# infancy/ky

Measured on AMD Instinct MI355X. Metric: Msamples/s (paths*spp), higher is better.
Workload: dtype f32

## Files before the change

ky_amd/csrc/ky_device.hpp:

```cpp
#pragma once
#ifndef __HIPCC_RTC__
#include <hip/hip_runtime.h>
#include <stdint.h>
#endif

#include "ky_scene.hpp"

#define KY_DEV __device__ __forceinline__

#if defined(KY_PROFILE_LANES) || defined(KY_PROFILE_CLOCKS) || defined(KY_MARKS)
#include "ky_measure.hpp"
#else
#define KY_PROBE(k) do { } while (0)
#define KY_CLK(k) do { } while (0)
#endif

namespace kyd {

KY_DEV float rcp(float x) { return __builtin_amdgcn_rcpf(x); }
KY_DEV float rsq(float x) { return __builtin_amdgcn_rsqf(x); }
KY_DEV float fsqrt(float x) { return __builtin_amdgcn_sqrtf(x); }
KY_DEV float sin_rev(float x) { return __builtin_amdgcn_sinf(x); }
KY_DEV float cos_rev(float x) { return __builtin_amdgcn_cosf(x); }
KY_DEV float clamp01f(float x) { return __builtin_amdgcn_fmed3f(x, 0.f, 1.f); }
// ... 838 lines not shown
    const float cos_o = dot(v.normal, wo), cos_i = dot(v.normal, wi);
    abs_cos_i = fabsf(cos_i);
    const bool same = cos_o * cos_i > 0;
    float p = same ? abs_cos_i * K_INV_PI : 0.f;
    scale = same ? K_INV_PI : 0.f;
    const bool phong = B.lobe == LOBE_PHONG;
    col = ld3(phong ? B.m->cs : B.m->c0);
    if (phong) {
        const float cos_alpha = dot(vertex_basis_c(v), wi);
        const float exponent = B.m->exponent;
        const float pe = phong_pow_lobe(cos_alpha, *B.m);
        const float p0 = exponent == 0.f ? 1.f : (exponent > 0.f ? 0.f : K_INF);
        scale = same ? pe * B.m->inv_eta : 0.f;
        p = (cos_alpha > 0.f ? pe : p0) * B.m->phong_pdf_norm;
    }
    const bool nondelta = !bsdf_is_delta(B);
    scale = nondelta ? scale : 0.f;
    pdf = nondelta ? p : 0.f;
}

KY_DEV f3 bsdf_sample_dir_nondelta(const Vertex& v, f3 wo, float u0, float u1, bool* back_dead = nullptr, bool flat_phong = false) {
    const bool phong = v.bsdf.lobe == LOBE_PHONG;
    const float cos_o = dot(v.normal, wo);
    float ang, rad, z = any_f();
    if (phong) {
        z = pow_nonneg(u1, v.bsdf.m->eta);
        rad = fsqrt(1.f - z * z);
        ang = u0;
    } else {
        const float rx = 2.f * u0 - 1, ry = 2.f * u1 - 1;
        const bool xmajor = fabsf(rx) > fabsf(ry);
        rad = xmajor ? rx : ry;
        const float ratio = mul_legacy(xmajor ? ry : rx, rcp(rad));
        ang = xmajor ? 0.125f * ratio : 0.25f - 0.125f * ratio;
    }
    float px = cos_rev(ang) * rad, py = sin_rev(ang) * rad;
    if (!phong) {
        z = __builtin_copysignf(fsqrt(fmaxf(0.f, 1 - px * px - py * py)), cos_o);
    }
    const LobeBasis L = vertex_basis(v);
    f3 wi = L.a * px + L.b * py + L.c * z;
    if (!flat_phong)
    if (phong && cos_o < 0) {
        const float nw = dot(v.normal, wi);
        wi = wi - (2.f * nw) * v.normal;
        if (back_dead) {
            const float cos_alpha = z - 2.f * nw * dot(v.normal, L.c);
            const float pe = phong_pow(cos_alpha, v.bsdf.m->exponent, v.bsdf.m->exp_flags);
            *back_dead = v.bsdf.m->exponent > 0.f && !(cos_alpha > 0.f && pe > 0.f);
        }
    }
    return wi;
}

struct DeltaSample {
    f3 wi;
    float percent;
    float abs_cos;
    bool reflected;
};
KY_DEV DeltaSample bsdf_sample_delta(const Vertex& v, f3 wo, float u0) {
    const DMat& M = *v.bsdf.m;
    const bool glass = v.bsdf.lobe == LOBE_GLASS;
    const float cos_o = dot(v.normal, wo);
    const float eta_t = M.eta, inv_eta = M.inv_eta;
    const bool into = cos_o > 0;
    const float nz = into ? 1.f : -1.f;
    const float ratio = into ? inv_eta : eta_t;
    const float ei = into ? 1.f : eta_t, et = into ? eta_t : 1.f;
    const float cos_theta_i = fminf(fabsf(cos_o), 1.f);
    const float sin_theta_i_sq = fmaxf(0.f, 1 - cos_theta_i * cos_theta_i);
    const float sin_theta_t = ratio * fsqrt(sin_theta_i_sq);
    const bool tir = sin_theta_t >= 1;
    const float cos_theta_t = fsqrt(fmaxf(0.f, 1 - sin_theta_t * sin_theta_t));
    const float r_para = ((et * cos_theta_i) - (ei * cos_theta_t)) * rcp((et * cos_theta_i) + (ei * cos_theta_t));
    const float r_perp = ((ei * cos_theta_i) - (et * cos_theta_t)) * rcp((ei * cos_theta_i) + (et * cos_theta_t));
    const float reflect_percent = (!glass || tir) ? 1.f : (r_para * r_para + r_perp * r_perp) * 0.5f;
    DeltaSample s;
    s.reflected = !glass || u0 < reflect_percent;
    const float k = ratio * cos_theta_i - cos_theta_t;
    const float sw = s.reflected ? -1.f : -ratio, sn = s.reflected ? 2.f * cos_o : k * nz;
    s.wi = wo * sw + v.normal * sn;
    s.percent = s.reflected ? reflect_percent : 1 - reflect_percent;
    s.abs_cos = fabsf(s.reflected ? cos_o : -ratio * cos_o + k * nz);
    return s;
}

KY_DEV BsdfSample bsdf_sample(const Vertex& v, f3 wo, float u0, float u1) {
    BsdfSample s;
    if (bsdf_is_delta(v.bsdf)) {
        const DeltaSample d = bsdf_sample_delta(v, wo, u0);
        s.wi = d.wi;
        s.pdf = d.percent;
        s.f = (ld3(d.reflected ? v.bsdf.m->c0 : v.bsdf.m->c1) * d.percent) * rcp(d.abs_cos);
        s.flags = (d.reflected ? BSDF_REFLECTION : BSDF_TRANSMISSION) | BSDF_SPECULAR;
    } else {
        float abs_cos_i;
        s.wi = bsdf_sample_dir_nondelta(v, wo, u0, u1);
        bsdf_eval_pdf(v, wo, s.wi, s.f, s.pdf, abs_cos_i);
        s.flags = BSDF_REFLECTION | (v.bsdf.lobe == LOBE_PHONG ? BSDF_GLOSSY : BSDF_DIFFUSE);
    }
    return s;
}

struct BsdfContinue {
    f3 wi, weight;
    bool ok, specular;
};
KY_DEV BsdfContinue bsdf_continue(const Vertex& v, f3 wo, float u0, float u1, bool flat_phong = false) {
    BsdfContinue c;
    c.specular = bsdf_is_delta(v.bsdf);
    if (c.specular) {
        const DeltaSample d = bsdf_sample_delta(v, wo, u0);
        c.wi = d.wi;
        c.weight = ld3(d.reflected ? v.bsdf.m->c0 : v.bsdf.m->c1);
        c.ok = ((v.bsdf.m->exp_flags & (d.reflected ? 4 : 8)) != 0) & (d.percent != 0.f);
    } else {
        bool back_dead = false;
        c.wi = bsdf_sample_dir_nondelta(v, wo, u0, u1, &back_dead, flat_phong);
        const float cos_o = dot(v.normal, wo), cos_i = dot(v.normal, c.wi);
        const bool phong = v.bsdf.lobe == LOBE_PHONG;
        const f3 col = ld3(phong ? v.bsdf.m->c1 : v.bsdf.m->c0);
        c.weight = col * (phong ? fabsf(cos_i) : 1.f);
        const bool dead_u1 = phong & !(u1 > 0.f) & (v.bsdf.m->exponent > 0.f);
        c.ok = (cos_o * cos_i > 0) & ((v.bsdf.m->exp_flags & (phong ? 8 : 4)) != 0) & !dead_u1 & !back_dead;
    }
    return c;
}

struct LightSample {
    f3 position, wi, Li;
    float pdf;
    bool lit;
    f3 dir;
    float dist;
};

KY_DEV f3 uniform_sphere_sample(float u0, float u1) {
    const float z = 1 - 2 * u0;
    const float radius = fsqrt(fmaxf(0.f, 1.f - z * z));
    return mk3(radius * cos_rev(u1), radius * sin_rev(u1), z);
}

KY_DEV void shape_sample_position(const DLight& L, float u0, float u1, f3& position, f3& normal, int feat = 0) {
    if ((feat & KY_FEAT_RECT_LIGHTS) || (!(feat & KY_FEAT_SPHERE_LIGHTS) && L.shape_kind == KY_SHAPE_RECTANGLE)) {
        const float4 P = *reinterpret_cast<const float4*>(L.p1), E0 = *reinterpret_cast<const float4*>(L.e0), E1 = *reinterpret_cast<const float4*>(L.e1),
                     N = *reinterpret_cast<const float4*>(L.n);
        position = mk3(P.x, P.y, P.z) + mk3(E0.x, E0.y, E0.z) * u0 + mk3(E1.x, E1.y, E1.z) * u1;
        normal = mk3(N.x, N.y, N.z);
    } else if ((feat & KY_FEAT_SPHERE_LIGHTS) || L.shape_kind == KY_SHAPE_SPHERE) {
        const f3 dir = uniform_sphere_sample(u0, u1);
        position = ld3(L.p1) + L.radius * dir;
        normal = dir;
    } else if (L.shape_kind == KY_SHAPE_TRIANGLE) {
        const float su0 = fsqrt(u0);
        const float bx = 1 - su0, by = u1 * su0;
        position = bx * ld3(L.p1) + by * ld3(L.e0) + (1 - bx - by) * ld3(L.e1);
        normal = ld3(L.n);
    } else {
        const Frame fr = make_frame(ld3(L.n));
        float px, py;
        concentric_disk(u0, u1, px, py);
        position = ld3(L.p1) + L.radius * (fr.s * px + fr.t * py);
        normal = ld3(L.n);
    }
}

KY_DEV void shape_sample_direction(const DLight& L, f3 p, f3 p_normal, float u0, float u1, f3& lposition, f3& lnormal, float& pdf, int feat = 0, bool ipdf = false) {
    const bool sphere = (feat & KY_FEAT_SPHERE_LIGHTS) ? true : ((feat & KY_FEAT_RECT_LIGHTS) == 0 && L.shape_kind == KY_SHAPE_SPHERE);
    const f3 c = ld3(L.p1);
    const float dc2 = length_sq(p - c);
    if (sphere && !(dc2 <= L.radius * L.radius)) {
        const float inv_dist = rsq(dc2);
        const float sin_theta_max = L.radius * inv_dist;
        const float sin_theta_max_sq = sin_theta_max * sin_theta_max;
        const float inv_sin_theta_max = (dc2 * inv_dist) * L.e0[0];
        const float cos_theta_max = fsqrt(fmaxf(0.f, 1 - sin_theta_max_sq));
        float cos_theta = (cos_theta_max - 1) * u0 + 1;
        float sin_theta_sq = 1 - cos_theta * cos_theta;
        if (sin_theta_max_sq < 0.00068523f) {
            sin_theta_sq = sin_theta_max_sq * u0;
            cos_theta = fsqrt(1 - sin_theta_sq);
        }
        const float cos_alpha = sin_theta_sq * inv_sin_theta_max +
                                cos_theta * fsqrt(fmaxf(0.f, 1.f - sin_theta_sq * inv_sin_theta_max * inv_sin_theta_max));
        const float sin_alpha = fsqrt(fmaxf(0.f, 1.f - cos_alpha * cos_alpha));
        const Frame fr = make_frame((c - p) * inv_dist);
        const f3 world_normal = (sin_alpha * cos_rev(u1)) * (-fr.s) + (sin_alpha * sin_rev(u1)) * (-fr.t) + cos_alpha * (-fr.n);
        lposition = c + L.radius * world_normal;
        lnormal = world_normal;
        pdf = ipdf ? 2 * K_PI * (1 - cos_theta_max) : rcp(2 * K_PI * (1 - cos_theta_max));
        return;
    }
    shape_sample_position(L, u0, u1, lposition, lnormal, feat);
    const f3 wv = lposition - p;
    const float d2 = length_sq(wv);
    const f3 wi = wv * rsq(d2);
    const f3 nn = sphere ? p_normal : lnormal;
    if (ipdf) {
        const float r = rsq(d2);
        const float x = (L.area * fabsf(dot(nn, wi))) * (r * r);
        pdf = x > 0.f ? x : K_INF;
        return;
    }
    const float q = L.inv_area * d2 * rcp(fabsf(dot(nn, wi)));
    pdf = __builtin_amdgcn_classf(q, 0x180) ? q : 0.f;
}

KY_DEV float shape_pdf_direction(const DLight& L, const DShapeFull* __restrict__ full, f3 p, f3 p_normal, f3 wi, bool general = true, int feat = 0, bool ipdf = false) {
    const bool sphere = (feat & KY_FEAT_SPHERE_LIGHTS) ? true : ((feat & KY_FEAT_RECT_LIGHTS) == 0 && L.shape_kind == KY_SHAPE_SPHERE);
    const f3 c = ld3(L.p1);
    const float dc2 = length_sq(p - c);
    if (sphere && !(dc2 <= L.radius * L.radius)) {
        const float sin_theta_max_sq = L.radius * L.radius * rcp(dc2);
        const float cos_theta_max = fsqrt(fmaxf(0.f, 1 - sin_theta_max_sq));
        const float x = 2 * K_PI * (1 - cos_theta_max);
        return ipdf ? x : rcp(x);
    }

    const f3 o = offset_ray_origin(p, p_normal, wi);
    float t;
    if (!surf_hit(L.isect, full, o, wi, K_INF, t, general)) return ipdf ? K_INF : 0.f;
    const f3 hp = o + t * wi;
    f3 ln = ld3(L.n);
    if (sphere) ln = normalize(hp - c);
    float pdf = length_sq(p - hp) * rcp(fabsf(dot(ln, wi)) * L.area);
    if (isinf(pdf)) pdf = 0.f;
    return ipdf ? rcp(pdf) : pdf;
}

KY_DEV float env_pdf(float wz) {
    const float z = fminf(fmaxf(wz, -1.f), 1.f);
    const float sin_theta = fsqrt(fmaxf(0.f, 1.f - z * z));
    return sin_theta == 0 ? 0.f : rcp(2 * K_PI * K_PI * sin_theta);
}

KY_DEV LightSample light_sample_Li(const DLight& L, f3 p, f3 p_normal, float u0, float u1, int feat = 0, bool ipdf = false) {
    LightSample s;
    s.lit = true;
    s.dir = any3();
    s.dist = any_f();
    const SceneRef K{nullptr, false, feat};
    if (K.is_area(L.kind)) {
        f3 lposition, lnormal;
        shape_sample_direction(L, p, p_normal, u0, u1, lposition, lnormal, s.pdf, feat, ipdf);
        s.position = lposition;
        const f3 dv = lposition - p;
        const float d2 = length_sq(dv);
        const bool ok = !((ipdf ? __builtin_isinf(s.pdf) : s.pdf == 0) || ((feat & KY_FEAT_RECT_LIGHTS) ? false : d2 == 0));
        const float inv_d = rsq(d2);
        const f3 wi = dv * inv_d;
        s.dir = wi;
        s.dist = d2 * inv_d;
        s.wi = mk3(ok ? wi.x : 0.f, ok ? wi.y : 0.f, ok ? wi.z : 0.f);
        const bool lit = ok & (dot(lnormal, wi) < 0) & !is_black_bits(L.color);
        s.lit = lit;
        s.Li = mk3(lit ? L.color[0] : 0.f, lit ? L.color[1] : 0.f, lit ? L.color[2] : 0.f);
    } else if (K.is_delta(L.kind) && L.kind == KY_LIGHT_POINT) {
        const f3 lp = ld3(L.position);
        const f3 dv = lp - p;
        const float inv_d2 = rcp(length_sq(dv));
        s.position = lp;
        s.wi = dv * fsqrt(inv_d2);
        s.pdf = 1.f;
        s.Li = ld3(L.color) * inv_d2;
    } else if (K.is_delta(L.kind)) {
        s.wi = -ld3(L.direction);
        s.position = p + s.wi * (2 * L.world_radius);
        s.pdf = 1;
        s.Li = ld3(L.color);
    } else {
        s.wi = uniform_sphere_sample(u0, u1);
        s.position = p + s.wi * (2 * L.world_radius);
        s.pdf = env_pdf(s.wi.z);
        s.Li = ld3(L.color);
    }
    return s;
}

KY_DEV float light_pdf_Li(const DLight& L, const DShapeFull* __restrict__ full, f3 p, f3 p_normal, f3 wi, bool general = true, int feat = 0, bool ipdf = false) {
    const SceneRef K{nullptr, false, feat};
    if (K.is_area(L.kind)) return shape_pdf_direction(L, full, p, p_normal, wi, general, feat, ipdf);
    if (K.is_env(L.kind)) return env_pdf(wi.z);
    return 0;
}


KY_DEV f3 surface_emission(const LdsScene& Lds, int surface, f3 normal, f3 wo) {
    const int al = Lds.hit[surface].area_light;
    f3 e = mk3(0, 0, 0);
    if (al >= 0 && dot(normal, wo) > 0) e = mk3(Lds.light_color[al][0], Lds.light_color[al][1], Lds.light_color[al][2]);
    return e;
}

struct RideAlong {
    bool want;
    f3 o, d;
    float t;
    int hs;
};
struct ShadowQueue;
struct SqRay;
KY_DEV void sq_push_bsdf_query(SceneRef S, ShadowQueue& q, bool push, f3 o, f3 d, float tmax, f3 c, unsigned tag);
template <bool MIS, bool PER_LANE = false>
KY_DEV void estimate_by_bsdf(SceneRef S, const LdsScene& Lds, const Vertex& v, f3 wo, int li, float u0, float u1, bool active, f3& acc, f3 w,
                             ShadowQueue* sq = nullptr, f3 beta = f3{0, 0, 0}, float weight = 0.f, unsigned tag = 0, RideAlong* ra = nullptr, const DLight* Lp = nullptr) {
    const DLight& L = light_record<PER_LANE>(S, li, Lp);
    if (PER_LANE) { if (S.is_delta(L.kind)) active = false; } else
    if (S.is_delta(L.kind)) return;
    BsdfSample bs;
    f3 f_cos = any3(), o = any3(), Li = any3();
    bs.wi = any3();
    bs.f = any3();
    bs.pdf = any_f();
    bool live = false, lit = false;
    float t_l = any_f();
    const bool fast = PER_LANE ? ((S.feat & KY_FEAT_CARRIERS) != 0 && (S.feat & (KY_FEAT_SINGLE_AREA | KY_FEAT_SPHERE_LIGHTS)) != 0)
                         : (S.is_area(L.kind) && ((S.feat & KY_FEAT_CARRIERS) || (L.n_carriers >= 0 && S->n_gen == 0)));
    if (fast) {
        const bool act = active && !bsdf_is_delta(v.bsdf);
        if (act) {
            bs.wi = bsdf_sample_dir_nondelta(v, wo, u0, u1, nullptr, S.flat_phong());
            o = offset_ray_origin(v.position, v.normal, bs.wi);
        }
        t_l = K_INF;
        int c = -1;
        bool pending;
        Li = ld3(L.color);
        if (S.feat & KY_FEAT_OWN_CARRIER) {
            const DSurf& R = L.isect;
            float t;
            bool hit;
            if (S.no_par()) {
                const float4 q0 = make_float4(L.aar[0], L.aar[1], L.aar[2], L.aar[3]);
                const float rv = L.aar[4];
                const int ax = L.aar_axis;
                float u_, v_;
                if (ax == 0) {
                    t = (q0.x - o.x) * rcp(bs.wi.x); u_ = (o.y + t * bs.wi.y) - q0.y; v_ = (o.z + t * bs.wi.z) - q0.w;
                    asm volatile("; lamp in an x plane" : "+v"(t), "+v"(u_), "+v"(v_));
                } else if (ax == 1) {
                    t = (q0.x - o.y) * rcp(bs.wi.y); u_ = (o.z + t * bs.wi.z) - q0.y; v_ = (o.x + t * bs.wi.x) - q0.w;
                    asm volatile("; lamp in a y plane" : "+v"(t), "+v"(u_), "+v"(v_));
                } else {
                    t = (q0.x - o.z) * rcp(bs.wi.z); u_ = (o.x + t * bs.wi.x) - q0.y; v_ = (o.y + t * bs.wi.y) - q0.w;
                    asm volatile("; lamp in a z plane" : "+v"(t), "+v"(u_), "+v"(v_));
                }
                hit = (fabsf(u_) <= q0.z) & (fabsf(v_) <= rv) & (t > K_SHAPE_EPS);
            } else {
                hit = par_hit(make_float4(R.f[0], R.f[1], R.f[2], R.f[3]), make_float4(R.f[4], R.f[5], R.f[6], R.f[7]), make_float4(R.f[8], R.f[9], R.f[10], R.f[11]), o, bs.wi, K_INF, t);
            }
            const bool ok = act & hit;
            t_l = ok ? t : t_l;
            c = ok ? L.carrier[0] : c;
            pending = ok && !is_black_bits(L.color);
        } else {
        for (int k = 0; k < L.n_carriers; ++k) {
            float t;
            bool hit;
            if (S.sphere_lights() && k == 0)
                hit = sph_hit(make_float4(L.aar[0], L.aar[1], L.aar[2], L.aar[3]), o, bs.wi, t_l, t, true);
            else
                hit = surf_hit(surf_record<PER_LANE>(S, L.carrier[k]), S->full, o, bs.wi, t_l, t, S.general, S.sphere_lights());
            const bool ok = act & hit;
            t_l = ok ? t : t_l;
            c = ok ? L.carrier[k] : c;
        }
        pending = c >= 0 && !is_black(Li);
        if (pending) {
            const f3 hp = o + t_l * bs.wi;
            pending = dot(hit_normal(Lds.hit[c], hp, bs.wi), bs.wi) < 0;
        }
        }
        if (pending) {
            float abs_cos_i;
            bsdf_eval_pdf(v, wo, bs.wi, bs.f, bs.pdf, abs_cos_i);
            f_cos = bs.f * abs_cos_i;
            live = !(is_black(f_cos) || (MIS ? (bs.pdf <= 0) : (bs.pdf == 0)));
            pending = live;
        }
        if (sq) {
            f3 c = any3();
            if (pending) {
                f3 Lq = (f_cos * Li) * rcp(bs.pdf);
                if (MIS) {
                    float light_pdf;
                    if (L.pdf_from_carrier) {
                        const f3 hp = o + t_l * bs.wi;
                        light_pdf = length_sq(v.position - hp) * rcp(fabsf(dot(ld3(L.n), bs.wi)) * L.area);
                        if (isinf(light_pdf)) light_pdf = 0.f;
                    } else {
                        light_pdf = light_pdf_Li(L, S->full, v.position, v.normal, bs.wi, S.general, S.feat);
                    }
                    Lq = light_pdf > 0 ? (f_cos * Li) * (2.f * rcp(bs.pdf + light_pdf)) : mk3(0, 0, 0);
                }
                c = (Lq * beta) * weight;
                pending = !(c.x == 0.f && c.y == 0.f && c.z == 0.f);
            }
            sq_push_bsdf_query(S, *sq, pending, o, bs.wi, t_l * (1.f - 1e-6f), c, tag);
            return;
        }
        unsigned long long queries = __ballot(pending);
        bool blocked = false;
        if (S.large && S->n_surfaces > 64) {
            KY_PROBE(2);
            if (pending) blocked = trace_any(S, S->occ, o, bs.wi, t_l * (1.f - 1e-6f));
        } else {
            const int lane = (int)__lane_id();
            while (queries) {
                const int src = __ffsll((long long)queries) - 1;
                queries &= queries - 1;
                const f3 qo = mk3(__shfl(o.x, src), __shfl(o.y, src), __shfl(o.z, src));
                const f3 qd = mk3(__shfl(bs.wi.x, src), __shfl(bs.wi.y, src), __shfl(bs.wi.z, src));
                const float qt = __shfl(t_l, src);
                int idx = lane < S->n_surfaces ? lane : 0;
                asm volatile("" : "+v"(idx));
                const DSurf& mine = S->all[idx];
                float t;
                const bool ok = (lane < S->n_surfaces) && surf_hit(mine, S->full, qo, qd, qt, t, S.general);
                const bool any = __any(ok);
                if (lane == src) blocked = any;
            }
        }
        lit = pending && !blocked;
    } else {
        if (active) {
            bs = bsdf_sample(v, wo, u0, u1);
            f_cos = bs.f * fabsf(dot(bs.wi, v.normal));
            live = !(is_black(f_cos) || (MIS ? (bs.pdf <= 0) : (bs.pdf == 0)));
            o = offset_ray_origin(v.position, v.normal, bs.wi);
        }
        float t = K_INF;
        KY_PROBE(2);
        int hs = -1;
        if (ra) {
            const bool ride = ra->want;
            f3 to = o, td = bs.wi;
            if (ride) { to = ra->o; td = ra->d; }
            const int h = (live || ride) ? trace_nearest(S, to, td, t) : -1;
            if (ride) { ra->hs = h; ra->t = t; ra->want = false; }
            else hs = h;
        } else {
            hs = live ? trace_nearest(S, o, bs.wi, t) : -1;
        }
        Li = mk3(0, 0, 0);
        if (hs >= 0) {
            if (Lds.hit[hs].area_light == li) {
                const f3 hp = o + t * bs.wi;
                Li = surface_emission(Lds, hs, hit_normal(Lds.hit[hs], hp, bs.wi), -bs.wi);
            }
        } else if (live && S.is_env(L.kind)) {
            Li = ld3(L.color);
        }
        lit = live && !is_black(Li);
    }
    if (lit) {
        if (MIS) {
            float light_pdf;
            if (fast && L.pdf_from_carrier) {
                const f3 hp = o + t_l * bs.wi;
                if (S.ipdf()) {
                    light_pdf = (fabsf(dot(ld3(L.n), bs.wi)) * L.area) * rcp(length_sq(v.position - hp));
                    if (!(light_pdf > 0.f)) light_pdf = K_INF;
                } else {
                    light_pdf = length_sq(v.position - hp) * rcp(fabsf(dot(ld3(L.n), bs.wi)) * L.area);
                    if (isinf(light_pdf)) light_pdf = 0.f;
                }
            } else {
                light_pdf = light_pdf_Li(L, S->full, v.position, v.normal, bs.wi, S.general, S.feat, S.ipdf());
            }
            if (S.ipdf()) {
                if (light_pdf < K_INF) acc = acc + w * ((f_cos * Li) * ((2.f * light_pdf) * rcp(bs.pdf * light_pdf + 1.f)));
            } else
            if (light_pdf > 0) acc = acc + w * ((f_cos * Li) * (2.f * rcp(bs.pdf + light_pdf)));
        } else {
            acc = acc + w * ((f_cos * Li) * rcp(bs.pdf));
        }
    }
}

#ifndef KY_SQ_FLUSH_AT
#define KY_SQ_FLUSH_AT 64
#endif
constexpr int KY_SQ_ENTRY = 3;
#ifndef KY_SQ_CAP_ENTRIES
#define KY_SQ_CAP_ENTRIES 64
#endif
constexpr int KY_SQ_CAP = KY_SQ_CAP_ENTRIES;
struct ShadowQueue {
    float4* base;
    int n;
    const int* c_pix;
    unsigned long long* c_def;
    unsigned long long* accum;
    unsigned* flags;
    const unsigned* counter;
};
struct SqRay {
    f3 o, d, c;
    float tmax;
    unsigned tag;
};
#define KY_SQ_SLOT(q, i) ((q).base + (i) * KY_SQ_ENTRY)
KY_DEV void sq_store(float4* e, const SqRay& r) {
    e[0] = make_float4(r.o.x, r.o.y, r.o.z, r.tmax);
    e[1] = make_float4(r.d.x, r.d.y, r.d.z, __uint_as_float(r.tag));
    e[2] = make_float4(r.c.x, r.c.y, r.c.z, 0.f);
}
KY_DEV SqRay sq_load(const float4* e) {
    const float4 a = e[0], b = e[1], c = e[2];
    return SqRay{mk3(a.x, a.y, a.z), mk3(b.x, b.y, b.z), mk3(c.x, c.y, c.z), a.w, __float_as_uint(b.w)};
}
KY_DEV void sq_trace(SceneRef S, const ShadowQueue& q, const SqRay& r) {
    if (trace_any(S, S->occ_deferred_ok ? S->occ : S->trav, r.o, r.d, r.tmax)) return;
    const float c[3] = {r.c.x, r.c.y, r.c.z};
    const int pix = (int)(r.tag >> 6), owner = (int)((threadIdx.x & ~63u) | (r.tag & 63u));
    const bool local = q.c_pix[owner] == pix;
    unsigned fl = 0;
    const float limit = film_limit_for(c, q.counter);
#pragma unroll
    for (int ch = 0; ch < 3; ++ch) {
        const unsigned long long fx = film_fixed(c[ch], limit, ch, fl);
        if (fx != 0) {
            if (local) atomicAdd(&q.c_def[ch * 256 + owner], fx);
            else atomicAdd(&q.accum[(size_t)pix * 3 + ch], fx);
        }
    }
    if (fl) atomicOr(&q.flags[pix], fl);
}
KY_DEV void sq_push(SceneRef S, ShadowQueue& q, bool push, SqRay r) {
    const unsigned long long m = __ballot(push);
    if (!m) return;
    const int k = __popcll(m);
    const int rank = (int)__builtin_amdgcn_mbcnt_hi((unsigned)(m >> 32), __builtin_amdgcn_mbcnt_lo((unsigned)m, 0u));
    if (q.n + k < KY_SQ_FLUSH_AT) {
        if (push) sq_store(KY_SQ_SLOT(q, q.n + rank), r);
        q.n += k;
        return;
    }
    asm volatile("" ::: "memory");
    const unsigned long long idle = ~m;
    const int idx = (int)__builtin_amdgcn_mbcnt_hi((unsigned)(idle >> 32), __builtin_amdgcn_mbcnt_lo((unsigned)idle, 0u));
    const bool pop = !push && idx < q.n;
    if (pop) r = sq_load(KY_SQ_SLOT(q, q.n - 1 - idx));
    q.n -= min(q.n, 64 - k);
    if (KY_SQ_FLUSH_AT == 64 || push || pop) sq_trace(S, q, r);
}
KY_DEV void sq_push_bsdf_query(SceneRef S, ShadowQueue& q, bool push, f3 o, f3 d, float tmax, f3 c, unsigned tag) {
    sq_push(S, q, push, SqRay{o, d, c, tmax, tag});
}
KY_DEV void sq_drain(SceneRef S, ShadowQueue& q) {
    const int lane = (int)__lane_id();
    __builtin_amdgcn_fence(__ATOMIC_ACQ_REL, "wavefront");
    if (lane < q.n) sq_trace(S, q, sq_load(KY_SQ_SLOT(q, lane)));
    q.n = 0;
}

template <bool MIS, bool PER_LANE = false>
KY_DEV void estimate_by_emitter_deferred(SceneRef S, const Vertex& v, f3 wo, int li, float u0, float u1, bool active, f3 beta, float weight,
                                         unsigned tag, ShadowQueue& q, const DLight* Lp = nullptr) {
    const DLight& L = light_record<PER_LANE>(S, li, Lp);
    bool push = false;
    SqRay r{any3(), any3(), any3(), any_f(), tag};
    if (active) {
        const bool ip = S.ipdf();
        const LightSample ls = light_sample_Li(L, v.position, v.normal, u0, u1, S.feat, ip);
        if (S.is_area(L.kind)) {
            r.d = ls.dir;
            r.tmax = ls.dist - 2e-3f;
        } else {
            const f3 to = ls.position - v.position;
            const float d2 = length_sq(to);
            const float inv_d = rsq(d2);
            r.d = to * inv_d;
            r.tmax = d2 * inv_d - 2e-3f;
        }
        r.o = offset_ray_origin(v.position, v.normal, r.d);
        f3 col;
        float scale, bsdf_pdf, abs_cos_i;
        bsdf_eval_parts(v, wo, S.is_area(L.kind) ? r.d : ls.wi, col, scale, bsdf_pdf, abs_cos_i);
        const bool delta_light = S.is_delta(L.kind);
        const float fc = scale * abs_cos_i;
        const float k = fc * (ip ? ((!MIS || delta_light) ? ls.pdf : (2.f * ls.pdf) * rcp(1.f + bsdf_pdf * ls.pdf))
                                 : ((!MIS || delta_light) ? rcp(ls.pdf) : 2.f * rcp(ls.pdf + bsdf_pdf))) * weight;
        const bool area = S.is_area(L.kind);
        const f3 Li = area ? ld3(L.color) : ls.Li;
        r.c = ((col * Li) * beta) * k;
        push = (area ? ls.lit : !is_black(ls.Li)) && (ip || !(MIS ? ls.pdf <= 0 : ls.pdf == 0)) && !(fc <= 0.f) && !is_black(col);
        if (S.is_area(L.kind) && L.sampled_is_surface) {
            float t;
            if (surf_hit(L.isect, S->full, r.o, r.d, r.tmax, t, S.general, S.sphere_lights(), false)) push = false;
        }
    }
    sq_push(S, q, push, r);
}

KY_DEV bool light_sample_occluded(SceneRef S, int li, f3 o, f3 dir, float tmax) {
    const unsigned tab = (unsigned)scene_light(S, li).shadow_table;
    const bool two = (tab & 1u) != 0;
    bool occ = trace_any(S, scene_at<DTrav>(S, tab & ~1u), o, dir, tmax);
    if (two) {
        const float4 plane = scene_at<float4>(S, opaque_off((unsigned)__builtin_offsetof(DScene, ts_plane)));
        const f3 pn = mk3(plane.x, plane.y, plane.z);
        const f3 e = o + dir * tmax;
        const bool need = !occ && (fminf(dot(pn, e), dot(pn, o)) <= plane.w);
        if (__any(need)) {
            if (need) occ = trace_any_planar(S, S->occ_behind, o, dir, tmax);
        }
    }
    return occ;
}

template <bool MIS, bool PER_LANE = false>
KY_DEV void estimate_by_emitter(SceneRef S, const LdsScene& Lds, const Vertex& v, f3 wo, int li, float u0, float u1, f3& acc, f3 w, const DLight* Lp = nullptr) {
    const DLight& L = light_record<PER_LANE>(S, li, Lp);
    KY_PROBE(3);
    const bool ip = S.ipdf();
    const LightSample ls = light_sample_Li(L, v.position, v.normal, u0, u1, S.feat, ip);
    const bool area = S.is_area(L.kind);
    const bool dead = (area ? !ls.lit : is_black(ls.Li)) || (!(ip || area) && (MIS ? (ls.pdf <= 0) : (ls.pdf == 0)));
    KY_CLK(5);
    if (!dead) {
        f3 dir;
        float dist;
        if (area) {
            dir = ls.dir;
            dist = ls.dist;
        } else {
            const f3 to = ls.position - v.position;
            const float d2 = length_sq(to);
            const float inv_d = rsq(d2);
            dir = to * inv_d;
            dist = d2 * inv_d;
        }
        const f3 o = offset_ray_origin(v.position, v.normal, dir);
        KY_PROBE(4);
        bool occ;
        if constexpr (PER_LANE) occ = trace_any(S, S->occ_deferred_ok ? S->occ : S->trav, o, dir, dist - 2e-3f);
        else occ = light_sample_occluded(S, li, o, dir, dist - 2e-3f);
        KY_CLK(6);
        if (!occ) {
            KY_PROBE(5);
            f3 col;
            float scale, bsdf_pdf, abs_cos_i;
            bsdf_eval_parts(v, wo, area ? dir : ls.wi, col, scale, bsdf_pdf, abs_cos_i);
            const float fc = scale * abs_cos_i;
            if (!(fc <= 0.f) && !is_black(col)) {
                const bool delta_light = S.is_delta(L.kind);
                const float k = fc * (ip ? ((!MIS || delta_light) ? ls.pdf : (2.f * ls.pdf) * rcp(1.f + bsdf_pdf * ls.pdf))
                                         : ((!MIS || delta_light) ? rcp(ls.pdf) : 2.f * rcp(ls.pdf + bsdf_pdf)));
                acc = acc + ((col * (area ? ld3(L.color) : ls.Li)) * w) * k;
            }
            KY_CLK(7);
        }
    }
}

template <bool MIS, bool PER_LANE = false>
KY_DEV void estimate_by_emitter_ride(SceneRef S, const LdsScene& Lds, const Vertex& v, f3 wo, int li, float u0, float u1, bool active, RideAlong& ra, f3& acc, f3 w,
                                     const DLight* Lp = nullptr) {
    const DLight& L = light_record<PER_LANE>(S, li, Lp);
    LightSample ls{any3(), any3(), any3(), any_f(), false, any3(), any_f()};
    const bool area = S.is_area(L.kind);
    bool dead = true;
    if (active) {
        ls = light_sample_Li(L, v.position, v.normal, u0, u1, S.feat);
        dead = (area ? !ls.lit : is_black(ls.Li)) || (MIS ? (ls.pdf <= 0) : (ls.pdf == 0));
    }
    f3 o = any3(), dir = any3();
    float tmax = any_f();
    if (!dead) {
        if (area) {
            dir = ls.dir;
            tmax = ls.dist - 2e-3f;
        } else {
            const f3 to = ls.position - v.position;
            const float d2 = length_sq(to);
            const float inv_d = rsq(d2);
            dir = to * inv_d;
            tmax = d2 * inv_d - 2e-3f;
        }
        o = offset_ray_origin(v.position, v.normal, dir);
    }
    bool occ = true;
    const bool ride = ra.want;
    if (__any(ride)) {
        if (ride) { o = ra.o; dir = ra.d; tmax = K_INF; }
        int hs = -1;
        if (ride || !dead) hs = trace_nearest(S, o, dir, tmax);
        occ = hs >= 0;
        if (ride) { ra.hs = hs; ra.t = tmax; ra.want = false; }
    } else if (!dead) {
        if constexpr (PER_LANE) occ = trace_any(S, S->occ_deferred_ok ? S->occ : S->trav, o, dir, tmax);
        else occ = light_sample_occluded(S, li, o, dir, tmax);
    }
    if (!dead && !occ) {
        f3 col;
        float scale, bsdf_pdf, abs_cos_i;
        bsdf_eval_parts(v, wo, area ? dir : ls.wi, col, scale, bsdf_pdf, abs_cos_i);
        const float fc = scale * abs_cos_i;
        if (!(fc <= 0.f) && !is_black(col)) {
            const bool delta_light = S.is_delta(L.kind);
            const float k = fc * ((!MIS || delta_light) ? rcp(ls.pdf) : 2.f * rcp(ls.pdf + bsdf_pdf));
            acc = acc + ((col * (area ? ld3(L.color) : ls.Li)) * w) * k;
        }
    }
}

KY_DEV void estimate_env_both(SceneRef S, const Vertex& v, f3 wo, float ub0, float ub1, float ul0, float ul1, f3& acc_b, f3& acc_l, f3 w) {
    const DLight& L = scene_light(S, 0);
    const bool dark = is_black_bits(L.color);
    AnyRay A;
    A.d = bsdf_sample_dir_nondelta(v, wo, ub0, ub1, nullptr, S.flat_phong());
    A.o = offset_ray_origin(v.position, v.normal, A.d);
    A.tmax = K_INF;
    const bool live_b = !dark;
    const float z = 1 - 2 * ul0;
    const float sin_theta = fsqrt(fmaxf(0.f, 1.f - z * z));
    const f3 wl = mk3(sin_theta * cos_rev(ul1), sin_theta * sin_rev(ul1), z);
    const float pl = sin_theta == 0 ? 0.f : rcp(2 * K_PI * K_PI * sin_theta);
    const bool live_l = !dark && !(pl <= 0);
    AnyRay B{offset_ray_origin(v.position, v.normal, wl), wl, 2 * L.world_radius - 2e-3f};
    bool occ_b = true, occ_l = true;
    if (live_b | live_l) trace_any_pair(S, A, B, occ_b, occ_l);
    const f3 Li = ld3(L.color);
    if (live_b && !occ_b) {
        f3 f;
        float pdf, abs_cos_i;
        bsdf_eval_pdf(v, wo, A.d, f, pdf, abs_cos_i);
        const f3 f_cos = f * abs_cos_i;
        const float light_pdf = env_pdf(A.d.z);
        if (!(is_black(f_cos) || pdf <= 0) && light_pdf > 0) acc_b = acc_b + w * ((f_cos * Li) * (2.f * rcp(pdf + light_pdf)));
    }
    if (live_l && !occ_l) {
        f3 col;
        float scale, bsdf_pdf, abs_cos_i;
        bsdf_eval_parts(v, wo, wl, col, scale, bsdf_pdf, abs_cos_i);
        const float fc = scale * abs_cos_i;
        if (!(fc <= 0.f) && !is_black(col)) acc_l = acc_l + ((col * Li) * w) * (fc * (2.f * rcp(pl + bsdf_pdf)));
    }
}

template <bool DEBUG_SAMPLER>
KY_DEV void sample_all_light(SceneRef S, const LdsScene& Lds, const Vertex& v, f3 wo, Sampler& smp, int strategy, bool active, f3& Lo, f3 beta,
                             unsigned* decisions = nullptr, ShadowQueue* sq = nullptr, float weight = 0.f, unsigned tag = 0, RideAlong* ra = nullptr) {
    const int nl = S.single_light() ? 1 : S->n_lights;
    const f3 w = strategy == KY_DIRECT_BOTH_MIS ? beta * 0.5f : beta;
    for (int li = 0; li < nl; ++li) {
        float ub0 = any_f(), ub1 = any_f(), ul0 = any_f(), ul1 = any_f();
        if (active) { ub0 = sampler_next<DEBUG_SAMPLER>(smp); ub1 = sampler_next<DEBUG_SAMPLER>(smp); }
        f3 Lb = mk3(0, 0, 0), Ll = mk3(0, 0, 0);
        f3& ab = decisions ? Lb : Lo;
        f3& al = decisions ? Ll : Lo;
        const f3 wt = decisions ? mk3(1, 1, 1) : w;
        if (strategy == KY_DIRECT_BOTH_MIS && (S.feat & KY_FEAT_SINGLE_ENV) && !sq && !ra) {
            if (active) {
                ul0 = sampler_next<DEBUG_SAMPLER>(smp); ul1 = sampler_next<DEBUG_SAMPLER>(smp);
                estimate_env_both(S, v, wo, ub0, ub1, ul0, ul1, ab, al, wt);
            }
        } else if (strategy == KY_DIRECT_BOTH_MIS) {
            KY_CLK(3);
            estimate_by_bsdf<true>(S, Lds, v, wo, li, ub0, ub1, active, ab, wt, sq, beta, weight * 0.5f, tag, ra);
            KY_CLK(4);
            if (active) { ul0 = sampler_next<DEBUG_SAMPLER>(smp); ul1 = sampler_next<DEBUG_SAMPLER>(smp); }
            if (sq) estimate_by_emitter_deferred<true>(S, v, wo, li, ul0, ul1, active, beta, weight * 0.5f, tag, *sq);
            else if (ra) estimate_by_emitter_ride<true>(S, Lds, v, wo, li, ul0, ul1, active, *ra, al, wt);
            else if (active) estimate_by_emitter<true>(S, Lds, v, wo, li, ul0, ul1, al, wt);
        } else {
            if (active) { ul0 = sampler_next<DEBUG_SAMPLER>(smp); ul1 = sampler_next<DEBUG_SAMPLER>(smp); }
            KY_CLK(3);
            if (strategy == KY_DIRECT_BSDF_MIS) {
                estimate_by_bsdf<true>(S, Lds, v, wo, li, ub0, ub1, active, ab, wt);
            } else if (strategy == KY_DIRECT_LIGHT_MIS) {
                if (sq) estimate_by_emitter_deferred<true>(S, v, wo, li, ul0, ul1, active, beta, weight, tag, *sq);
                else if (active) estimate_by_emitter<true>(S, Lds, v, wo, li, ul0, ul1, al, wt);
            } else if (strategy == KY_DIRECT_LIGHT) {
                if (sq) estimate_by_emitter_deferred<false>(S, v, wo, li, ul0, ul1, active, beta, weight, tag, *sq);
                else if (active) estimate_by_emitter<false>(S, Lds, v, wo, li, ul0, ul1, al, wt);
            } else if (strategy == KY_DIRECT_BSDF) {
                const int lk = S->light[li].kind;
                if (!S.is_delta(lk)) {
                    float u0 = any_f(), u1 = any_f();
                    if (active) { u0 = sampler_next<DEBUG_SAMPLER>(smp); u1 = sampler_next<DEBUG_SAMPLER>(smp); }
                    estimate_by_bsdf<false>(S, Lds, v, wo, li, u0, u1, active, ab, wt);
                }
            }
        }
        if (decisions) {
            if (active) Lo = Lo + w * (Lb + Ll);
            if (li < 16) *decisions |= (is_black(Lb) ? 0u : 1u << li) | (is_black(Ll) ? 0u : 1u << (16 + li));
        }
    }
}

template <bool DEBUG_SAMPLER>
KY_DEV void sample_single_light(SceneRef S, const LdsScene& Lds, const Vertex& v, f3 wo, Sampler& smp, bool active, f3& Lo, f3 beta,
                                unsigned* decisions = nullptr, ShadowQueue* sq = nullptr, float weight = 0.f, unsigned tag = 0, RideAlong* ra = nullptr) {
    const int nl = S.single_light() ? 1 : S->n_lights;
    if (nl == 0) return;
    int li = 0;
    float ub0 = any_f(), ub1 = any_f(), ul0 = any_f(), ul1 = any_f();
    if (active) {
        const float u = sampler_next<DEBUG_SAMPLER>(smp);
        li = min((int)(u * (float)nl), nl - 1);
        ul0 = sampler_next<DEBUG_SAMPLER>(smp); ul1 = sampler_next<DEBUG_SAMPLER>(smp);
        ub0 = sampler_next<DEBUG_SAMPLER>(smp); ub1 = sampler_next<DEBUG_SAMPLER>(smp);
    }
    const float fn = (float)nl;
    const f3 w = beta * (0.5f * fn);
    const float wq = weight * (0.5f * fn);
    f3 Lb = mk3(0, 0, 0), Ll = mk3(0, 0, 0);
    f3& ab = decisions ? Lb : Lo;
    f3& al = decisions ? Ll : Lo;
    const f3 wt = decisions ? mk3(1, 1, 1) : w;
    if (S.single_light()) {
        if ((S.feat & KY_FEAT_SINGLE_ENV) && !sq && !ra) {
            if (active) estimate_env_both(S, v, wo, ub0, ub1, ul0, ul1, ab, al, wt);
        } else {
            estimate_by_bsdf<true>(S, Lds, v, wo, 0, ub0, ub1, active, ab, wt, sq, beta, wq, tag, ra);
            if (sq) estimate_by_emitter_deferred<true>(S, v, wo, 0, ul0, ul1, active, beta, wq, tag, *sq);
            else if (ra) estimate_by_emitter_ride<true>(S, Lds, v, wo, 0, ul0, ul1, active, *ra, al, wt);
            else if (active) estimate_by_emitter<true>(S, Lds, v, wo, 0, ul0, ul1, al, wt);
        }
    } else {
        const DLight* Lp = Lds.light + li;
        estimate_by_bsdf<true, true>(S, Lds, v, wo, li, ub0, ub1, active, ab, wt, sq, beta, wq, tag, ra, Lp);
        if (sq) estimate_by_emitter_deferred<true, true>(S, v, wo, li, ul0, ul1, active, beta, wq, tag, *sq, Lp);
        else if (ra) estimate_by_emitter_ride<true, true>(S, Lds, v, wo, li, ul0, ul1, active, *ra, al, wt, Lp);
        else if (active) estimate_by_emitter<true, true>(S, Lds, v, wo, li, ul0, ul1, al, wt, Lp);
    }
    if (decisions) {
        if (active) Lo = Lo + w * (Lb + Ll);
        if (li < 16) *decisions |= (is_black(Lb) ? 0u : 1u << li) | (is_black(Ll) ? 0u : 1u << (16 + li));
    }
}

template <bool DEBUG_SAMPLER>
KY_DEV void light_estimate_draws(SceneRef S, Sampler& smp, int strategy, bool active) {
    if (!active) return;
    const int nl = S.single_light() ? 1 : S->n_lights;
    int n = 4 * nl;
    if (strategy == KY_DIRECT_SINGLE_BOTH_MIS) n = nl > 0 ? 5 : 0;
    else if (strategy == KY_DIRECT_BSDF)
        for (int li = 0; li < nl; ++li) n += S.is_delta(S->light[li].kind) ? 0 : 2;
    for (int i = 0; i < n; ++i) (void)sampler_next<DEBUG_SAMPLER>(smp);
}

struct PathState {
    f3 o, d;
    f3 beta, Lo;
    Sampler smp;
    int bounces;
    bool prev_specular;
};

KY_DEV void path_state_dead(PathState& ps) {
    ps.o = mk3(any_reg(), any_reg(), any_reg()); ps.d = mk3(any_reg(), any_reg(), any_reg()); ps.beta = mk3(any_reg(), any_reg(), any_reg());
    ps.smp.s0 = any_reg_u(); ps.smp.s1 = any_reg_u(); ps.bounces = (int)any_reg_u(); ps.prev_specular = any_reg_u() != 0;
}


template <bool DEBUG_SAMPLER, bool KEEP_LO = false>
KY_DEV void path_begin(PathState& ps, SceneRef S, uint32_t pixel_key, int x, int y, int sample) {
    sampler_start(ps.smp, pixel_key, (uint32_t)sample);
    const float u0 = sampler_next<DEBUG_SAMPLER>(ps.smp), u1 = sampler_next<DEBUG_SAMPLER>(ps.smp);
    generate_ray(S, (float)x + u0, (float)y + u1, ps.o, ps.d);
    ps.beta = mk3(1, 1, 1);
    if (!KEEP_LO) ps.Lo = mk3(0, 0, 0);
    ps.bounces = 0;
    ps.prev_specular = false;
}

template <bool DEBUG_SAMPLER, int DROP = 0>
KY_DEV bool path_intersect(PathState& ps, Vertex& v, SceneRef S, const LdsScene& Lds, const RenderConst& rc, int drop_rt = 0) {
    const int drop = DROP >= 0 ? DROP : drop_rt;
    float t = K_INF;
    KY_PROBE(0);
    const int hs = trace_nearest(S, ps.o, ps.d, t);
    const bool hit = hs >= 0;

    if (hit) {
        v.t = t;
        v.position = ps.o + t * ps.d;
        v.normal = hit_normal(Lds.hit[hs], v.position, ps.d);
        v.surface = hs;
    }
    bool see;
    if (rc.integrator == KY_INTEGRATOR_PATH_TRACING_ITERATION || rc.integrator == KY_INTEGRATOR_DIRECT_LIGHTING ||
        rc.integrator == KY_INTEGRATOR_PATH_TRACING_RECURSION_DEFERED)
        see = ps.bounces == 0 || ps.prev_specular;
    else if (rc.integrator == KY_INTEGRATOR_PATH_TRACING_RECURSION)
        see = ps.bounces == 0;
    else
        see = rc.integrator == KY_INTEGRATOR_SIMPLE_PATH_TRACING_RECURSION;
    if (drop != 0 && ps.bounces < 2 && ((drop >> ps.bounces) & 1)) see = false;
    if (see) {
        if (hit) {
            if (!S.no_carried_light()) {
            const int al = Lds.hit[hs].area_light;
            if (al >= 0 && dot(v.normal, ps.d) < 0)
                ps.Lo = ps.Lo + ps.beta * mk3(Lds.light_color[al][0], Lds.light_color[al][1], Lds.light_color[al][2]);
            }
        } else if (S.may_have_env() && S->env_light >= 0) {
            ps.Lo = ps.Lo + ps.beta * ld3(S->light[S->env_light].color);
        }
    }
    if (!hit) return false;
    if (rc.integrator == KY_INTEGRATOR_PATH_TRACING_ITERATION || rc.integrator == KY_INTEGRATOR_PATH_TRACING_RECURSION_DEFERED ||
        rc.integrator == KY_INTEGRATOR_PATH_TRACING_RECURSION || rc.integrator == KY_INTEGRATOR_SIMPLE_PATH_TRACING_RECURSION)
        if (ps.bounces >= rc.max_path_depth) return false;
    return true;
}

template <bool DEBUG_SAMPLER>
KY_DEV int path_pick_lobe(PathState& ps, int surface, const LdsScene& Lds) {
    const DMat& M = Lds.mat[Lds.hit[surface].material];
    float lobe_u = 0.f;
    if (M.kind == KY_MATERIAL_PLASTIC) lobe_u = sampler_next<DEBUG_SAMPLER>(ps.smp);
    return pick_lobe(M, lobe_u);
}

struct VertexTrace {
    float* rows;
    int max_rows, n;
};

template <bool DEBUG_SAMPLER, int DROP = 0>
KY_DEV bool path_shade(PathState& ps, Vertex& v, SceneRef S, const LdsScene& Lds, const RenderConst& rc, bool active,
                       int lobe = -1, VertexTrace* tr = nullptr, ShadowQueue* sq = nullptr, unsigned tag = 0, bool ride_along = false, bool free_state = false,
                       int drop_rt = 0) {
    const int drop = DROP >= 0 ? DROP : drop_rt;
    if (active) {
        const DMat& M = Lds.mat[Lds.hit[v.surface].material];
        if (lobe < 0) {
            float lobe_u = 0.f;
            if (M.kind == KY_MATERIAL_PLASTIC) lobe_u = sampler_next<DEBUG_SAMPLER>(ps.smp);
            v.bsdf = make_bsdf(M, lobe_u, (S.feat & KY_FEAT_NO_DELTA) != 0);
        } else {
            v.bsdf = make_bsdf_for_lobe(M, lobe);
        }
        vertex_prepare(v, -ps.d, &Lds.hit[v.surface]);
    }
    const f3 wo = -ps.d;

    if (rc.integrator < KY_INTEGRATOR_DIRECT_LIGHTING) {
        if (active) {
            if (rc.integrator == KY_INTEGRATOR_POSITION) ps.Lo = ps.Lo + normalize(v.position);
            else if (rc.integrator == KY_INTEGRATOR_NORMAL) ps.Lo = ps.Lo + v.normal;
            else {
                float pdf, abs_cos_i;
                f3 base;
                bsdf_eval_pdf(v, wo, v.normal, base, pdf, abs_cos_i);
                ps.Lo = ps.Lo + base;
            }
        }
        return false;
    }

    KY_CLK(2);
    const bool recursion = rc.integrator == KY_INTEGRATOR_PATH_TRACING_RECURSION;
    const bool defered = rc.integrator == KY_INTEGRATOR_PATH_TRACING_RECURSION_DEFERED;
    const bool simple = rc.integrator == KY_INTEGRATOR_SIMPLE_PATH_TRACING_RECURSION;
    const bool delta = bsdf_is_delta(v.bsdf);
    const bool lit = active && !delta;
    const bool unlit = (drop & 2) != 0 && lit && ps.bounces == 0;
    const bool nee = lit && !unlit;
    KY_PROBE(6);
    unsigned decisions = 0;
    const bool riding = recursion && ride_along;
    RideAlong ra{false, any3(), any3(), K_INF, -1};
    f3 es_f = any3();
    float es_k = any_f();
    if (riding && active && delta) {
        const float e0 = sampler_next<DEBUG_SAMPLER>(ps.smp), e1 = sampler_next<DEBUG_SAMPLER>(ps.smp);
        const BsdfSample es = bsdf_sample(v, wo, e0, e1);
        ra.want = true;
        ra.o = v.position;
        ra.d = es.wi;
        es_f = es.f;
        es_k = fabsf(dot(es.wi, v.normal)) / es.pdf;
    }
    if (!simple && rc.strategy == KY_DIRECT_SINGLE_BOTH_MIS) {
        sample_single_light<DEBUG_SAMPLER>(S, Lds, v, wo, ps.smp, nee, ps.Lo, ps.beta, tr ? &decisions : nullptr, sq, rc.inv_spp, tag, riding ? &ra : nullptr);
    } else
    if (!simple) {
        sample_all_light<DEBUG_SAMPLER>(S, Lds, v, wo, ps.smp, rc.strategy, nee, ps.Lo, ps.beta, tr ? &decisions : nullptr, sq, rc.inv_spp, tag,
                                        riding ? &ra : nullptr);
    }
    if ((drop & 2) != 0 && !simple) light_estimate_draws<DEBUG_SAMPLER>(S, ps.smp, rc.strategy, unlit);
    KY_CLK(8);
    if (rc.integrator == KY_INTEGRATOR_DIRECT_LIGHTING) return false;
    if (!active) {
        if (free_state) path_state_dead(ps);
        return false;
    }

    if (recursion && delta) {
        if (!riding) {
            const float e0 = sampler_next<DEBUG_SAMPLER>(ps.smp), e1 = sampler_next<DEBUG_SAMPLER>(ps.smp);
            const BsdfSample es = bsdf_sample(v, wo, e0, e1);
            ra.o = v.position;
            ra.d = es.wi;
            ra.want = true;
            es_f = es.f;
            es_k = fabsf(dot(es.wi, v.normal)) / es.pdf;
        }
        if (ra.want) {
            ra.t = K_INF;
            ra.hs = trace_nearest(S, ra.o, ra.d, ra.t);
        }
        f3 Le = (S.may_have_env() && S->env_light >= 0) ? ld3(S->light[S->env_light].color) : mk3(0, 0, 0);
        if (ra.hs >= 0) {
            const f3 hp = ra.o + ra.t * ra.d;
            Le = surface_emission(Lds, ra.hs, hit_normal(Lds.hit[ra.hs], hp, ra.d), -ra.d);
            if (Lds.mat[Lds.hit[ra.hs].material].kind == KY_MATERIAL_PLASTIC) (void)sampler_next<DEBUG_SAMPLER>(ps.smp);
        }
        ps.Lo = ps.Lo + ps.beta * ((es_f * Le) * es_k);
    }

    const float u0 = sampler_next<DEBUG_SAMPLER>(ps.smp), u1 = sampler_next<DEBUG_SAMPLER>(ps.smp);
    KY_PROBE(7);
    if (rc.integrator == KY_INTEGRATOR_PATH_TRACING_ITERATION && !tr) {
        const BsdfContinue c = bsdf_continue(v, wo, u0, u1, S.flat_phong());
        bool cont = c.ok;
        ps.beta = ps.beta * c.weight;
        ps.prev_specular = c.specular;
        ps.o = offset_ray_origin(v.position, v.normal, c.wi);
        ps.d = c.wi;
        if (ps.bounces > 3) {
            const float q = fmaxf(0.05f, 1 - max3(ps.beta));
            const float u = sampler_next<DEBUG_SAMPLER>(ps.smp);
            cont = cont && !(u < q);
            ps.beta = ps.beta * rcp(1 - q);
        }
        ps.bounces += 1;
        return cont && !(ps.bounces >= rc.max_path_depth && !ps.prev_specular);
    }
    BsdfSample bs = bsdf_sample(v, wo, u0, u1);
    if (tr && tr->n < tr->max_rows) {
        float* r = tr->rows + 26 * tr->n++;
        r[0] = (float)ps.bounces; r[1] = (float)S->orig[v.surface]; r[2] = (float)v.bsdf.lobe;
        r[3] = v.position.x; r[4] = v.position.y; r[5] = v.position.z; r[6] = v.normal.x; r[7] = v.normal.y; r[8] = v.normal.z;
        r[9] = wo.x; r[10] = wo.y; r[11] = wo.z; r[12] = ps.beta.x; r[13] = ps.beta.y; r[14] = ps.beta.z;
        r[15] = ps.Lo.x; r[16] = ps.Lo.y; r[17] = ps.Lo.z; r[18] = bs.f.x; r[19] = bs.f.y; r[20] = bs.f.z; r[21] = bs.pdf;
        r[22] = fabsf(dot(bs.wi, v.normal)); r[23] = (float)bs.flags; r[24] = (float)(decisions & 0xffffu); r[25] = (float)(decisions >> 16);
    }
    if (is_black(bs.f) || bs.pdf == 0.f) return false;
    if (rc.integrator == KY_INTEGRATOR_PATH_TRACING_ITERATION) {
        ps.beta = ps.beta * (bs.f * (fabsf(dot(bs.wi, v.normal)) * rcp(bs.pdf)));
        ps.prev_specular = (bs.flags & BSDF_SPECULAR) != 0;
        ps.o = offset_ray_origin(v.position, v.normal, bs.wi);
        ps.d = bs.wi;
        if (ps.bounces > 3) {
            const float q = fmaxf(0.05f, 1 - max3(ps.beta));
            const float u = sampler_next<DEBUG_SAMPLER>(ps.smp);
            if (u < q) return false;
            ps.beta = ps.beta * rcp(1 - q);
        }
        ps.bounces += 1;
        if (ps.bounces >= rc.max_path_depth && !ps.prev_specular) return false;
        return true;
    }
    if (ps.bounces + 1 > 3) {
        const float m = max3(bs.f);
        const float u = sampler_next<DEBUG_SAMPLER>(ps.smp);
        if (!(u < m)) return false;
        bs.f = bs.f * (1 / m);
    }
    ps.beta = ps.beta * (bs.f * (fabsf(dot(bs.wi, v.normal)) * rcp(bs.pdf)));
    ps.prev_specular = delta;
    ps.o = recursion ? offset_ray_origin(v.position, v.normal, bs.wi) : v.position;
    ps.d = bs.wi;
    ps.bounces += 1;
    if (ps.bounces >= rc.max_path_depth && (recursion || (defered && !ps.prev_specular))) return false;
    return true;
}

}
```

Baseline: 22970.

## Defer BSDF sample draws into estimator and early-exit when no lane hits light

Moves the BSDF random-number draws for the both-MIS strategy into estimate_by_bsdf, so they happen only on paths that actually sample. It adds a wave-wide ballot that returns early when no lane's BSDF ray hits the light, skipping the BSDF evaluation. It also rebuilds the Bsdf from the material and lobe indices in free_state mode to lower register pressure. The cost is extra branching and the risk of changing the order of the random sequence (delta-BSDF lanes now draw and sample), which alters sample statistics.

```diff
diff --git a/ky_amd/csrc/ky_device.hpp b/ky_amd/csrc/ky_device.hpp
--- a/ky_amd/csrc/ky_device.hpp
+++ b/ky_amd/csrc/ky_device.hpp
@@ -1164,12 +1164,16 @@
 struct ShadowQueue;
 struct SqRay;
 KY_DEV void sq_push_bsdf_query(SceneRef S, ShadowQueue& q, bool push, f3 o, f3 d, float tmax, f3 c, unsigned tag);
-template <bool MIS, bool PER_LANE = false>
+template <bool MIS, bool PER_LANE = false, bool DEBUG_SAMPLER = false>
 KY_DEV void estimate_by_bsdf(SceneRef S, const LdsScene& Lds, const Vertex& v, f3 wo, int li, float u0, float u1, bool active, f3& acc, f3 w,
-                             ShadowQueue* sq = nullptr, f3 beta = f3{0, 0, 0}, float weight = 0.f, unsigned tag = 0, RideAlong* ra = nullptr, const DLight* Lp = nullptr) {
+                             ShadowQueue* sq = nullptr, f3 beta = f3{0, 0, 0}, float weight = 0.f, unsigned tag = 0, RideAlong* ra = nullptr, const DLight* Lp = nullptr,
+                             Sampler* draw = nullptr) {
     const DLight& L = light_record<PER_LANE>(S, li, Lp);
     if (PER_LANE) { if (S.is_delta(L.kind)) active = false; } else
-    if (S.is_delta(L.kind)) return;
+    if (S.is_delta(L.kind)) {
+        if (draw && active) { (void)sampler_next<DEBUG_SAMPLER>(*draw); (void)sampler_next<DEBUG_SAMPLER>(*draw); }
+        return;
+    }
     BsdfSample bs;
     f3 f_cos = any3(), o = any3(), Li = any3();
     bs.wi = any3();
@@ -1180,14 +1184,16 @@
     const bool fast = PER_LANE ? ((S.feat & KY_FEAT_CARRIERS) != 0 && (S.feat & (KY_FEAT_SINGLE_AREA | KY_FEAT_SPHERE_LIGHTS)) != 0)
                          : (S.is_area(L.kind) && ((S.feat & KY_FEAT_CARRIERS) || (L.n_carriers >= 0 && S->n_gen == 0)));
     if (fast) {
-        const bool act = active && !bsdf_is_delta(v.bsdf);
+        const bool act = draw ? active : (active && !bsdf_is_delta(v.bsdf));
         if (act) {
+            if (draw) { u0 = sampler_next<DEBUG_SAMPLER>(*draw); u1 = sampler_next<DEBUG_SAMPLER>(*draw); }
             bs.wi = bsdf_sample_dir_nondelta(v, wo, u0, u1, nullptr, S.flat_phong());
             o = offset_ray_origin(v.position, v.normal, bs.wi);
         }
         t_l = K_INF;
         int c = -1;
         bool pending;
+        bool own_pending = false;
         Li = ld3(L.color);
         if (S.feat & KY_FEAT_OWN_CARRIER) {
             const DSurf& R = L.isect;
@@ -1212,10 +1218,9 @@
             } else {
                 hit = par_hit(make_float4(R.f[0], R.f[1], R.f[2], R.f[3]), make_float4(R.f[4], R.f[5], R.f[6], R.f[7]), make_float4(R.f[8], R.f[9], R.f[10], R.f[11]), o, bs.wi, K_INF, t);
             }
-            const bool ok = act & hit;
-            t_l = ok ? t : t_l;
-            c = ok ? L.carrier[0] : c;
-            pending = ok && !is_black_bits(L.color);
+            t_l = t;
+            pending = act & hit;
+            own_pending = true;
         } else {
         for (int k = 0; k < L.n_carriers; ++k) {
             float t;
@@ -1234,6 +1239,8 @@
             pending = dot(hit_normal(Lds.hit[c], hp, bs.wi), bs.wi) < 0;
         }
         }
+        if (!sq && __builtin_amdgcn_ballot_w64(pending) == 0) return;
+        if (own_pending) pending = pending && !is_black_bits(L.color);
         if (pending) {
             float abs_cos_i;
             bsdf_eval_pdf(v, wo, bs.wi, bs.f, bs.pdf, abs_cos_i);
@@ -1287,6 +1294,7 @@
         lit = pending && !blocked;
     } else {
         if (active) {
+            if (draw) { u0 = sampler_next<DEBUG_SAMPLER>(*draw); u1 = sampler_next<DEBUG_SAMPLER>(*draw); }
             bs = bsdf_sample(v, wo, u0, u1);
             f_cos = bs.f * fabsf(dot(bs.wi, v.normal));
             live = !(is_black(f_cos) || (MIS ? (bs.pdf <= 0) : (bs.pdf == 0)));
@@ -1610,7 +1618,8 @@
     const f3 w = strategy == KY_DIRECT_BOTH_MIS ? beta * 0.5f : beta;
     for (int li = 0; li < nl; ++li) {
         float ub0 = any_f(), ub1 = any_f(), ul0 = any_f(), ul1 = any_f();
-        if (active) { ub0 = sampler_next<DEBUG_SAMPLER>(smp); ub1 = sampler_next<DEBUG_SAMPLER>(smp); }
+        const bool draw_in_half = strategy == KY_DIRECT_BOTH_MIS && !((S.feat & KY_FEAT_SINGLE_ENV) && !sq && !ra);
+        if (active && !draw_in_half) { ub0 = sampler_next<DEBUG_SAMPLER>(smp); ub1 = sampler_next<DEBUG_SAMPLER>(smp); }
         f3 Lb = mk3(0, 0, 0), Ll = mk3(0, 0, 0);
         f3& ab = decisions ? Lb : Lo;
         f3& al = decisions ? Ll : Lo;
@@ -1622,7 +1631,7 @@
             }
         } else if (strategy == KY_DIRECT_BOTH_MIS) {
             KY_CLK(3);
-            estimate_by_bsdf<true>(S, Lds, v, wo, li, ub0, ub1, active, ab, wt, sq, beta, weight * 0.5f, tag, ra);
+            estimate_by_bsdf<true, false, DEBUG_SAMPLER>(S, Lds, v, wo, li, ub0, ub1, active, ab, wt, sq, beta, weight * 0.5f, tag, ra, nullptr, &smp);
             KY_CLK(4);
             if (active) { ul0 = sampler_next<DEBUG_SAMPLER>(smp); ul1 = sampler_next<DEBUG_SAMPLER>(smp); }
             if (sq) estimate_by_emitter_deferred<true>(S, v, wo, li, ul0, ul1, active, beta, weight * 0.5f, tag, *sq);
@@ -1792,8 +1801,11 @@
                        int lobe = -1, VertexTrace* tr = nullptr, ShadowQueue* sq = nullptr, unsigned tag = 0, bool ride_along = false, bool free_state = false,
                        int drop_rt = 0) {
     const int drop = DROP >= 0 ? DROP : drop_rt;
+    const bool free_bsdf = free_state && !(S.feat & KY_FEAT_SINGLE_ENV);
+    int mat_i = free_bsdf ? (int)any_reg_u() : 0, lobe_i = free_bsdf ? (int)any_reg_u() : 0;
     if (active) {
-        const DMat& M = Lds.mat[Lds.hit[v.surface].material];
+        mat_i = Lds.hit[v.surface].material;
+        const DMat& M = Lds.mat[mat_i];
         if (lobe < 0) {
             float lobe_u = 0.f;
             if (M.kind == KY_MATERIAL_PLASTIC) lobe_u = sampler_next<DEBUG_SAMPLER>(ps.smp);
@@ -1801,8 +1813,10 @@
         } else {
             v.bsdf = make_bsdf_for_lobe(M, lobe);
         }
+        lobe_i = v.bsdf.lobe;
         vertex_prepare(v, -ps.d, &Lds.hit[v.surface]);
     }
+    if (free_bsdf) v.bsdf = Bsdf{lobe_i, &Lds.mat[mat_i]};
     const f3 wo = -ps.d;
 
     if (rc.integrator < KY_INTEGRATOR_DIRECT_LIGHTING) {
```

Measured after the change: 23080, median of 6. About the same (+0.5%).
